# JuliaParallel/DistributedArrays.jl

Measured on NVIDIA H100. Metric: GB/s for map! and sum on Float32 DArray, higher is better.
Workload: dtype f32

## Files before the change

### distributedarrays.jl_b200/_broadcast.py

```python
from __future__ import annotations

import ctypes as C
import struct
from typing import Callable, List, Optional, Sequence, Tuple

import numpy as np

from builtins import any as builtins_any

from . import _lib
from ._darray import B200Array, DArray, dab_dtype, darray, makelocal
from .layout import shape_of
from .runtime import close_remote_reads, open_remote_reads, runtime

_RANK = {"bool": 0, "i32": 1, "i64": 2, "i128": 3, "f16": 4, "f32": 5, "f64": 6}


class _TagTypes(dict):

    def __missing__(self, tag):
        raise _lib.UnsupportedError(_lib.ERR_UNSUPPORTED, f"values of type {tag} have no array element type on the GPU backend "
                                    "(Int128 is served as the value type of mapreduce(f, op, d) only)")


_NPT = _TagTypes({"bool": np.dtype(np.bool_), "i32": np.dtype(np.int32), "i64": np.dtype(np.int64), "f32": np.dtype(np.float32),
                  "f64": np.dtype(np.float64), "c64": np.dtype(np.complex64), "c128": np.dtype(np.complex128),
                  "f16": np.dtype(np.float16)})
_TAG = {v: k for k, v in _NPT.items()}
SLICE_TRACING = [0]
_CT = {"bool": "bool", "i32": "int", "i64": "long long", "i128": "i128", "f32": "float", "f64": "double", "c64": "jl_c64", "c128": "jl_c128",
       "f16": "jl_f16"}
_COMP = {"c64": "f32", "c128": "f64"}
_CPLX_OF = {"f32": "c64", "f64": "c128"}


def _jl_name(t: str) -> str:
    return {"bool": "Bool", "i32": "Int32", "i64": "Int64", "i128": "Int128", "f16": "Float16", "f32": "Float32", "f64": "Float64"}.get(t, t)


def is_ctag(t: str) -> bool:
    return t in _COMP


def tag_of(dtype) -> str:
    dt = np.dtype(dtype)
    if dt not in _TAG:
        raise _lib.UnsupportedError(_lib.ERR_UNSUPPORTED, f"element type {dt} not served by the GPU backend")
    return _TAG[dt]


def promote(a: str, b: str) -> str:
    if a == b:
        return a
    if is_ctag(a) or is_ctag(b):
        if "i128" in (a, b):
            raise _lib.UnsupportedError(_lib.ERR_UNSUPPORTED, "Int128 values mixed with complex values are not served")
# ... 746 lines not shown
    if isinstance(a, np.ndarray) and a.ndim > 0:
        view = _bcview(a.shape, I)
        sl = a[tuple(slice(lo - 1, hi) for lo, hi in view)]
        return LocalArg(B200Array.from_numpy(rt, sl), None, tag_of(a.dtype), temp=True)
    e = Expr.wrap(a.item() if isinstance(a, np.ndarray) else a)
    return LocalArg(None, e.val, e.jt)


def _remote_args(dest_layout, args) -> List[DArray]:
    return [a for a in args if isinstance(a, DArray) and not (a.layout.pids == dest_layout.pids and a.layout.indices == dest_layout.indices)]


def _broadcast_chunks(dest: DArray, expr: Expr, args) -> DArray:
    rt = dest.rt
    fenced = open_remote_reads(rt, _remote_args(dest.layout, args), "host")
    for pid, out in dest.chunks.items():
        I = dest.layout.localindices(pid)
        largs = [_localise(rt, a, I, pid) for a in args]
        run_local(rt, expr, out, largs)
        for la in largs:
            if la.temp and la.arr is not None:
                la.arr.free()
    close_remote_reads(rt, fenced, "host")
    return dest


def _materialise_views(args):
    from ._darray import SubDArray
    out, temps = [], []
    for a in args:
        if isinstance(a, SubDArray):
            a = a.to_darray()
            temps.append(a)
        out.append(a)
    return out, temps


def broadcast_into(dest: DArray, f: Callable, *args) -> DArray:
    args, _views = _materialise_views(args)
    try:
        return _broadcast_into(dest, f, *args)
    finally:
        for v in _views:
            v.close()


def _broadcast_into(dest: DArray, f: Callable, *args) -> DArray:
    shapes = [a.dims if isinstance(a, DArray) else (a.shape if isinstance(a, np.ndarray) else ()) for a in args]
    for shp in shapes:
        for k, s in enumerate(shp):
            want = dest.dims[k] if k < len(dest.dims) else 1
            if s != 1 and s != want:
                raise _lib.DimensionMismatch(_lib.ERR_DIM_MISMATCH, f"destination axes {dest.dims} are not compatible with source axes {tuple(shp)}")
    expr = trace(f, [_arg_tag(a) for a in args])
    return _broadcast_chunks(dest, expr, args)


def broadcast(f: Callable, *args, rt=None) -> DArray:
    args, _views = _materialise_views(args)
    try:
        return _broadcast(f, *args, rt=rt)
    finally:
        for v in _views:
            v.close()


def _broadcast(f: Callable, *args, rt=None) -> DArray:
    rt = rt or next((a.rt for a in args if isinstance(a, DArray)), None) or runtime()
    shapes = [a.dims if isinstance(a, DArray) else (a.shape if isinstance(a, np.ndarray) else ()) for a in args]
    dims = _bc_shape(shapes)
    expr = trace(f, [_arg_tag(a) for a in args])
    out_dt = _NPT[expr.jt]
    dest = darray(lambda I: B200Array.empty(rt, shape_of(I), out_dt), dims, dtype=out_dt, rt=rt)
    return _broadcast_chunks(dest, expr, args)


def copy(d: DArray) -> DArray:
    from ._darray import similar
    return _broadcast_into(similar(d), lambda x: x, d)


deepcopy = copy


def drandn(dims, procs=None, dist=None, dtype=np.float64, seed: int = 1234, rt=None) -> DArray:
    from ._darray import component_dtype, drand
    dt = np.dtype(dtype)
    if dt.kind == "c":
        ct = component_dtype(dt)
        re = drandn(dims, procs, dist, dtype=ct, seed=seed, rt=rt)
        im = drandn(dims, procs, dist, dtype=ct, seed=seed + 2, rt=rt)
        from ._darray import darray_like
        out = darray_like(lambda I: B200Array.empty(re.rt, shape_of(I), dt), re, dtype=dt)
        _broadcast_into(out, lambda a, b: complex_(0.7071067811865476 * a, 0.7071067811865476 * b), re, im)
        re.close()
        im.close()
        return out
    if dt == np.dtype(np.float16):
        from ._darray import darray_like
        d64 = drandn(dims, procs, dist, dtype=np.float64, seed=seed, rt=rt)
        out = darray_like(lambda I: B200Array.empty(d64.rt, shape_of(I), dt), d64, dtype=dt)
        _broadcast_into(out, Float16, d64)
        d64.close()
        return out
    if dt.kind != "f":
        raise _lib.UnsupportedError(_lib.ERR_UNSUPPORTED, f"drandn of eltype {dt}")
    u1 = drand(dims, procs, dist, dtype=dt, seed=seed, rt=rt)
    u2 = drand(dims, procs, dist, dtype=dt, seed=seed + 1, rt=rt)
# ... 48 lines not shown
```

### distributedarrays.jl_b200/_darray.py

```python
from __future__ import annotations

import ctypes as C
import itertools
import weakref
from typing import Callable, Dict, List, Optional, Sequence, Tuple

import numpy as np

from . import _lib
from .layout import Layout, Range, default_procs, layout_from_chunk_shapes, make_layout, rlen, shape_of, slab_plan
from .runtime import Runtime, close_remote_reads, open_remote_reads, runtime

_DT = {np.dtype(np.float32): _lib.F32, np.dtype(np.float64): _lib.F64, np.dtype(np.int32): _lib.I32,
       np.dtype(np.int64): _lib.I64, np.dtype(np.bool_): _lib.U8,
       np.dtype(np.complex64): _lib.C64, np.dtype(np.complex128): _lib.C128,
       np.dtype(np.float16): _lib.F16}
_NP = {_lib.F32: np.dtype(np.float32), _lib.F64: np.dtype(np.float64), _lib.I32: np.dtype(np.int32),
       _lib.I64: np.dtype(np.int64), _lib.U8: np.dtype(np.bool_), _lib.C64: np.dtype(np.complex64), _lib.C128: np.dtype(np.complex128),
       _lib.F16: np.dtype(np.float16)}


def dab_dtype(dt) -> int:
    dt = np.dtype(dt)
    if dt not in _DT:
        raise _lib.UnsupportedError(_lib.ERR_UNSUPPORTED, f"element type {dt} is not served by the GPU backend (no host fallback)")
    return _DT[dt]


def np_dtype(code: int) -> np.dtype:
    return _NP[code]


def is_complex(dt) -> bool:
    return np.dtype(dt).kind == "c"


def component_dtype(dt) -> np.dtype:
    dt = np.dtype(dt)
    return {np.dtype(np.complex64): np.dtype(np.float32), np.dtype(np.complex128): np.dtype(np.float64)}.get(dt, dt)


def refuse_float16(what: str, *xs):
    for x in xs:
        x = getattr(x, "parent", x) if not hasattr(x, "dtype") else x
        dt = getattr(x, "dtype", None)
        if dt is not None and np.dtype(dt) == np.dtype(np.float16):
            raise _lib.UnsupportedError(_lib.ERR_UNSUPPORTED, f"{what} of Float16 data is not served (no Float16 kernel; no host fallback)")


_allowscalar = [True]


def allowscalar(flag: bool = True):
    _allowscalar[0] = bool(flag)


class B200Array:

    __slots__ = ("rt", "ptr", "shape", "dtype", "_own", "_keep", "_temp")

    def __init__(self, rt: Runtime, ptr: int, shape: Sequence[int], dtype, own: bool = True, keep=None, temp: bool = False):
        self.rt, self.ptr, self.shape, self.dtype = rt, int(ptr), tuple(int(s) for s in shape), np.dtype(dtype)
        self._own, self._keep, self._temp = own, keep, temp

    @classmethod
    def empty(cls, rt: Runtime, shape: Sequence[int], dtype, temp: bool = False) -> "B200Array":
        dtype = np.dtype(dtype)
        n = int(np.prod(shape)) if len(shape) else 1
        ptr = rt.alloc_temp(n * dtype.itemsize) if temp else rt.alloc(n * dtype.itemsize)
        return cls(rt, ptr, shape, dtype, temp=temp)

    @classmethod
    def from_numpy(cls, rt: Runtime, a: np.ndarray) -> "B200Array":
        a = np.asarray(a)
        dab_dtype(a.dtype)
        out = cls.empty(rt, a.shape, a.dtype)
        out.copy_from_host(a)
        return out

    @property
    def size(self) -> int:
        return int(np.prod(self.shape)) if len(self.shape) else 1

    @property
    def nbytes(self) -> int:
        return self.size * self.dtype.itemsize

    @property
    def ndim(self) -> int:
        return len(self.shape)

    def copy_from_host(self, a: np.ndarray, sync: bool = True):
        a = np.asarray(a, dtype=self.dtype)
        if tuple(a.shape) != self.shape:
            raise _lib.DimensionMismatch(_lib.ERR_DIM_MISMATCH, f"host array {a.shape} vs chunk {self.shape}")
        if self.size == 0:
            return
        if not a.flags.f_contiguous:
            if a.ndim == 2 and a.strides[0] == a.itemsize and a.strides[1] > 0:
                _lib.call("dab_h2d_2d", self.rt.ctx, C.c_void_p(self.ptr), a.shape[0] * a.itemsize, C.c_void_p(a.ctypes.data),
                          a.strides[1], a.shape[0] * a.itemsize, a.shape[1])
                if sync:
                    self.rt.sync()
                return
            a = np.asfortranarray(a)
        _lib.call("dab_h2d", self.rt.ctx, C.c_void_p(self.ptr), C.c_void_p(a.ctypes.data), self.nbytes)
        if sync:
            self.rt.sync()

    def to_numpy(self) -> np.ndarray:
        out = np.empty(self.shape, dtype=self.dtype, order="F")
        if self.size:
            _lib.call("dab_d2h", self.rt.ctx, C.c_void_p(out.ctypes.data), C.c_void_p(self.ptr), self.nbytes)
            self.rt.sync()
        return out

    def free(self):
        if self._own and self.ptr:
            if self._temp:
                self.rt.free_temp(self.ptr)
            else:
                self.rt.free(self.ptr)
        self.ptr = 0

    def __repr__(self):
        return f"B200Array({self.dtype}, {self.shape}, ptr=0x{self.ptr:x}, dev={self.rt.device})"


def pinned_empty(rt: Runtime, shape, dtype) -> np.ndarray:
    dtype = np.dtype(dtype)
    n = int(np.prod(shape)) if len(shape) else 1
    p = C.c_void_p()
    _lib.call("dab_host_alloc", rt.ctx, max(1, n * dtype.itemsize), C.byref(p))
    buf = (C.c_char * max(1, n * dtype.itemsize)).from_address(p.value)
    arr = np.frombuffer(buf, dtype=dtype, count=n).reshape(shape, order="F")
# ... 655 lines not shown
```

### distributedarrays.jl_b200/_mapreduce.py

```python
from __future__ import annotations

import builtins
import ctypes as C
import operator
from itertools import accumulate
from typing import Callable, Dict, Optional, Sequence, Tuple

import numpy as np

from . import _lib
from ._broadcast import Expr, broadcast, is_ctag, tag_of, trace, _NPT
from ._darray import B200Array, DArray, component_dtype, dab_dtype, is_complex, np_dtype
from .layout import Layout, ravel, reduction_passes, shape_of, unravel
from .runtime import close_remote_reads, deliver, exchange_stacks, open_remote_reads

_OPS = {"+": _lib.SUM, "add": _lib.SUM, "sum": _lib.SUM, "*": _lib.PROD, "mul": _lib.PROD, "prod": _lib.PROD, "max": _lib.MAX,
        "min": _lib.MIN}
_OPF = {operator.add: _lib.SUM, operator.mul: _lib.PROD, builtins.max: _lib.MAX, builtins.min: _lib.MIN, np.add: _lib.SUM,
        np.multiply: _lib.PROD, np.maximum: _lib.MAX, np.minimum: _lib.MIN}


def _op_code(op) -> int:
    if isinstance(op, str) and op in _OPS:
        return _OPS[op]
    if op in _OPF:
        return _OPF[op]
    raise _lib.UnsupportedError(_lib.ERR_UNSUPPORTED, f"reduction operator {op!r} is not served by a kernel (no host fallback)")


_CMPMAP = {"eq": _lib.MAP_EQ, "ne": _lib.MAP_NE, "lt": _lib.MAP_LT, "le": _lib.MAP_LE, "gt": _lib.MAP_GT, "ge": _lib.MAP_GE}
_FLIP = {"lt": "gt", "le": "ge", "gt": "lt", "ge": "le", "eq": "eq", "ne": "ne"}


def classify_map(f: Optional[Callable], dtype) -> Tuple[Optional[int], Optional[np.ndarray], Optional[Expr]]:
    if f is None:
        return _lib.MAP_ID, None, None
    tag = tag_of(dtype)
    e = trace(f, [tag])
    if e.op == "arg":
        return _lib.MAP_ID, None, e
    if is_ctag(tag):
        if len(e.args) == 1 and e.args[0].op == "arg":
            code = {"abs": _lib.MAP_ABS, "abs2": _lib.MAP_ABS2, "neg": _lib.MAP_NEG, "isnan": _lib.MAP_ISNAN}.get(e.op)
            if code is not None:
                return code, None, e
        return None, None, e
    if e.jt == tag and len(e.args) == 1 and e.args[0].op == "arg":
        code = {"abs": _lib.MAP_ABS, "abs2": _lib.MAP_ABS2, "neg": _lib.MAP_NEG}.get(e.op)
        if code is not None:
            return code, None, e
    if e.op == "mul" and e.jt == tag and builtins.all(a.op == "arg" for a in e.args):
        return _lib.MAP_ABS2, None, e
    if e.op in _CMPMAP:
        l, r = e.args

        def unpromote(side, const):
            if side.op == "convert" and side.args[0].op == "arg" and side.args[0].jt == tag and const.op == "const":
                c = const.val
                if tag in ("f32", "f16") and const.jt == "f64" and float(_NPT[tag].type(c)) == c:
                    return side.args[0], Expr("const", (), tag, c)
                if tag in ("i32", "i64") and const.jt in ("i64",) and side.jt == "i64":
                    return side.args[0], Expr("const", (), tag, c) if -2**31 <= c < 2**31 or tag == "i64" else (side, const)
            return side, const

        l, r = unpromote(l, r)
        r, l = unpromote(r, l)
        if l.op == "arg" and r.op == "const" and l.jt == tag:
            return _CMPMAP[e.op], np.asarray(r.val, dtype=np.dtype(dtype)), e
        if r.op == "arg" and l.op == "const" and r.jt == tag:
            return _CMPMAP[_FLIP[e.op]], np.asarray(l.val, dtype=np.dtype(dtype)), e
    if e.op == "isnan" and e.args[0].op == "arg":
        return _lib.MAP_ISNAN, None, e
    return None, None, e


def _result_dtype(dtype, op: int, mapc: int) -> np.dtype:
    out = C.c_int32()
    _lib.check(_lib.lib().dab_reduce_result_dtype(dab_dtype(dtype), op, mapc, C.byref(out)))
    return np.dtype(np.int64) if out.value == _lib.I64 else np_dtype(out.value)




def _gather_slots(d: DArray, launch: Callable[[int, B200Array, int], None]) -> np.ndarray:
    rt = d.rt
    wpr = rt.workers_per_rank
    slots = B200Array.empty(rt, (16 * wpr,), np.uint8, temp=True)
    try:
        for pid, ch in d.chunks.items():
            launch(pid, ch, slots.ptr + 16 * ((pid - 1) % wpr))
        if rt.world > 1:
            allslots = B200Array.empty(rt, (16 * wpr * rt.world,), np.uint8, temp=True)
            _lib.call("dab_allgather", rt.ctx, C.c_void_p(slots.ptr), C.c_void_p(allslots.ptr), 16 * wpr)
            host = allslots.to_numpy()
            allslots.free()
        else:
            host = slots.to_numpy()
    finally:
        rt.sync()
        slots.free()
    return host.view(np.uint8)


def _fold(host: np.ndarray, pids: Sequence[int], rdt: np.dtype, op: int):
    vals = np.empty(len(pids), dtype=rdt)
    for i, pid in enumerate(pids):
        vals[i] = host[16 * (pid - 1):16 * (pid - 1) + rdt.itemsize].view(rdt)[0]
    out = np.zeros(1, dtype=rdt)
    rcode = _lib.I64 if rdt == np.dtype(np.int64) else dab_dtype(rdt)
    _lib.check(_lib.lib().dab_combine_ordered(rcode, op, C.c_void_p(vals.ctypes.data), len(pids), C.c_void_p(out.ctypes.data)))
    return out[0], vals


def _int128(b: bytes) -> int:
    return int.from_bytes(b, "little", signed=True)


def wrap128(v: int) -> int:
    v &= (1 << 128) - 1
    return v - (1 << 128) if v >> 127 else v


def fold128(vals: Sequence[int], op: int) -> int:
    acc = vals[0]
    for v in vals[1:]:
        acc = wrap128(acc + v) if op == _lib.SUM else wrap128(acc * v) if op == _lib.PROD else (max(acc, v) if op == _lib.MAX else min(acc, v))
    return acc


def _check_nonempty(d: DArray, opc: int):
    if opc in (_lib.MAX, _lib.MIN):
        for pid in d.layout.pids:
# ... 45 lines not shown
        if ch.size == 0:
            return _empty_slot(rt, opc, np.dtype(np.int64) if wide else rdt, slot_ptr)
        I = d.layout.localindices(pid)
        largs = [_localise(rt, a, I, pid) for a in args]
        e, largs = split_c128_scalars(expr, largs)
        if len(largs) > 8:
            raise _lib.UnsupportedError(_lib.ERR_UNSUPPORTED, "more than 8 mapreduce arguments (a ComplexF64 scalar counts twice) are not served")
        src = codegen(e).encode()
        n = len(largs)
        dts = (C.c_int32 * n)(*[dab_dtype(NPT[la.tag]) for la in largs])
        ptrs = (C.c_void_p * n)(*[la.arr.ptr if la.arr is not None else None for la in largs])
        scal = (C.c_uint64 * n)()
        for k, la in enumerate(largs):
            if la.arr is None:
                scal[k] = int.from_bytes(np.asarray(la.scalar, dtype=NPT[la.tag]).tobytes().ljust(8, b"\0"), "little")
            elif la.temp:
                temps.append(la.arr)
        _lib.call("dab_mapreduce_expr", rt.ctx, src, val_code, opc_k, ch.size, n, dts, ptrs, scal, C.c_void_p(slot_ptr))

    try:
        host = _gather_slots(d, launch)
    finally:
        for t in temps:
            t.free()
        close_remote_reads(rt, fenced, "host")
    if wide:
        vals = [_int128(host[16 * (pid - 1):16 * pid].tobytes()) for pid in d.layout.pids]
        res = fold128(vals, opc)
        return (res, vals) if return_partials else res
    res, vals = _fold(host, d.layout.pids, rdt, opc if opc != _lib.COUNT else _lib.SUM)
    return (res, vals) if return_partials else res


def _mapreduce_all(f, op, d: DArray, return_partials: bool = False, others: Sequence = ()):
    opc = op if isinstance(op, int) else _op_code(op)
    if others:
        expr = trace(f, [tag_of(d.dtype)] + [_arg_tag_of(a) for a in others])
        return _mapreduce_expr(expr, opc, d, others, return_partials)
    mapc, param, expr = classify_map(f, d.dtype)
    if is_complex(d.dtype) and mapc is not None and not _complex_served(opc, mapc):
        if mapc == _lib.MAP_ID and opc in (_lib.MAX, _lib.MIN):
            raise TypeError(f"MethodError: no method matching isless(::{d.dtype}, ::{d.dtype}) -- complex numbers are not ordered")
        mapc = None
        if expr is None:
            expr = trace(lambda z: z, [tag_of(d.dtype)])
    if mapc is None:
        return _mapreduce_expr(expr, opc, d, (), return_partials)
    _check_nonempty(d, opc)
    rt = d.rt
    pp = C.c_void_p(param.ctypes.data) if param is not None else None
    rdt = _result_dtype(d.dtype, opc, mapc)
    if rt.workers_per_rank == 1 and d.layout.pids == rt.workers() and not return_partials:
        ch = d.chunks[rt.myid()]
        out = np.zeros(2, dtype=np.uint64)
        _lib.call("dab_mapreduce_all", rt.ctx, dab_dtype(d.dtype), opc, mapc, pp, C.c_void_p(ch.ptr), ch.size, C.c_void_p(out.ctypes.data))
        return out.view(np.uint8)[:rdt.itemsize].view(rdt)[0]
    code = dab_dtype(d.dtype)
    host = _gather_slots(d, lambda pid, ch, slot: _lib.call("dab_reduce", rt.ctx, code, opc, mapc, pp, C.c_void_p(ch.ptr), ch.size, C.c_void_p(slot)))
    res, vals = _fold(host, d.layout.pids, rdt, opc)
    return (res, vals) if return_partials else res


def _complex_served(opc: int, mapc: int) -> bool:
    out = C.c_int32()
    return _lib.lib().dab_reduce_result_dtype(_lib.C64, opc, mapc, C.byref(out)) == _lib.OK


def _arg_tag_of(a) -> str:
    from ._broadcast import _arg_tag
    return _arg_tag(a)


def reduce(op, d: DArray, dims=None, init=None):
    return mapreduce(None, op, d, dims=dims, init=init)


def mapreduce(f: Optional[Callable], op, d: DArray, *ds, dims=None, init=None, _partials: bool = False):
    from ._darray import SubDArray
    if isinstance(d, Expr):
        from . import _slices
        if _slices.tracing():
            return _slices.reduce_of_slice(f, op, d, ds, dims, init)
    if isinstance(d, SubDArray):
        tmp = d.to_darray()
        try:
            return mapreduce(f, op, tmp, *ds, dims=dims, init=init, _partials=_partials)
        finally:
            if dims is None:
                tmp.close()
    if dims is None:
        if init is not None:
            raise _lib.UnsupportedError(_lib.ERR_UNSUPPORTED, "mapreduce(f, op, d; init) without dims falls back to scalar iteration in the reference; not served")
        return _mapreduce_all(f, op, d, _partials, ds)
    if ds:
        tmp = broadcast(f, d, *ds)
        try:
            return mapreducedim(None, op, tmp, dims, init)
        finally:
            tmp.close()
    return mapreducedim(f, op, d, dims, init)


def sum(d: DArray, f: Optional[Callable] = None, dims=None):
    return mapreduce(f, "+", d, dims=dims)


def prod(d: DArray, f: Optional[Callable] = None, dims=None):
    return mapreduce(f, "*", d, dims=dims)


def maximum(d: DArray, f: Optional[Callable] = None, dims=None):
    return mapreduce(f, "max", d, dims=dims)


def minimum(d: DArray, f: Optional[Callable] = None, dims=None):
    return mapreduce(f, "min", d, dims=dims)


def _pred_reduce(opc: int, d: DArray, f: Optional[Callable]):
    from ._darray import SubDArray
    if isinstance(d, SubDArray):
        tmp = d.to_darray()
        try:
            return _pred_reduce(opc, tmp, f)
        finally:
            tmp.close()
    if f is None:
        if d.dtype != np.dtype(np.bool_):
            raise TypeError("TypeError: non-boolean used in boolean context")
        return _mapreduce_all(None, opc, d)
    mapc, param, e = classify_map(f, d.dtype)
# ... 343 lines not shown
```

### distributedarrays.jl_b200/csrc/dab_comm.cu

```cuda
#include <dlfcn.h>
#include <nccl.h>

#include "dab_common.cuh"
#include "dab_scalar_ops.cuh"

namespace {

struct NcclApi {
    void* handle = nullptr;
    ncclResult_t (*GetUniqueId)(ncclUniqueId*) = nullptr;
    ncclResult_t (*CommInitRank)(ncclComm_t*, int, ncclUniqueId, int) = nullptr;
    ncclResult_t (*CommDestroy)(ncclComm_t) = nullptr;
    ncclResult_t (*AllGather)(const void*, void*, size_t, ncclDataType_t, ncclComm_t, cudaStream_t) = nullptr;
    ncclResult_t (*AllReduce)(const void*, void*, size_t, ncclDataType_t, ncclRedOp_t, ncclComm_t, cudaStream_t) = nullptr;
    ncclResult_t (*Send)(const void*, size_t, ncclDataType_t, int, ncclComm_t, cudaStream_t) = nullptr;
    ncclResult_t (*Recv)(void*, size_t, ncclDataType_t, int, ncclComm_t, cudaStream_t) = nullptr;
    ncclResult_t (*GroupStart)() = nullptr;
    ncclResult_t (*GroupEnd)() = nullptr;
    const char* (*GetErrorString)(ncclResult_t) = nullptr;
    const char* (*GetLastError)(ncclComm_t) = nullptr;
    bool ok = false;
    char why[256] = "";
};

// ... 70 lines not shown
            __threadfence_system();
            break;
        }
    }
    __threadfence_system();
}

template <typename T>
__global__ void __launch_bounds__(256) accumulate_stack_kernel(T* __restrict__ y, size_t n, T beta, int beta_mode, T alpha, int alpha_one,
                                                              const T* __restrict__ stack, size_t stride, int count) {
    for (size_t i = (size_t)blockIdx.x * 256 + threadIdx.x; i < n; i += (size_t)gridDim.x * 256) {
        T v = beta_mode == 0 ? T(0) : (beta_mode == 1 ? y[i] : jl::mul(y[i], beta));
        for (int j = 0; j < count; ++j) {
            const T r = stack[(size_t)j * stride + i];
            v = jl::add(v, alpha_one ? r : jl::mul(alpha, r));
        }
        y[i] = v;
    }
}

}

extern "C" {

int32_t dab_comm_unique_id(void* id128) {
    NEED_NCCL(nullptr);
    if (!id128) return dab_fail(nullptr, DAB_ERR_ARG, "null id");
    static_assert(sizeof(ncclUniqueId) == 128, "ncclUniqueId is 128 bytes");
    ncclUniqueId id;
    DAB_NCCL(nullptr, api.GetUniqueId(&id));
    memcpy(id128, &id, 128);
    return DAB_OK;
}

int32_t dab_comm_init_rank(dab_ctx* ctx, const void* id128, int32_t rank, int32_t nranks) {
    DAB_ENTER(ctx);
    NEED_NCCL(ctx);
    DAB_REQUIRE(ctx, id128 && nranks >= 1 && rank >= 0 && rank < nranks && nranks <= DAB_MAX_RANKS, DAB_ERR_ARG,
                "dab_comm_init_rank: bad rank %d / nranks %d", rank, nranks);
    DAB_REQUIRE(ctx, !ctx->comm, DAB_ERR_ARG, "communicator already initialised");
    ncclUniqueId id;
    memcpy(&id, id128, 128);
    ncclComm_t comm;
    DAB_NCCL(ctx, api.CommInitRank(&comm, nranks, id, rank));
    ctx->comm = (void*)comm;
    ctx->rank = rank;
    ctx->nranks = nranks;
    return DAB_OK;
}

int32_t dab_comm_destroy(dab_ctx* ctx) {
    if (!ctx || !ctx->comm) return DAB_OK;
    NcclApi& api = nccl();
    cudaSetDevice(ctx->device);
    const int32_t st = dab_flush_pending(ctx);
    cudaStreamSynchronize(ctx->stream);
    if (api.ok) api.CommDestroy((ncclComm_t)ctx->comm);
    ctx->comm = nullptr;
    ctx->rank = 0;
    ctx->nranks = 1;
    return st;
}

int32_t dab_allgather(dab_ctx* ctx, const void* send_dev, void* recv_dev, size_t nbytes_per_rank) {
    DAB_ENTER(ctx);
    NEED_COMM(ctx);
    DAB_NCCL(ctx, api.AllGather(send_dev, recv_dev, nbytes_per_rank, ncclInt8, (ncclComm_t)ctx->comm, ctx->stream));
    ctx->launches++;
    return DAB_OK;
}

int32_t dab_allreduce(dab_ctx* ctx, int32_t dtype, int32_t op, const void* send_dev, void* recv_dev, size_t count) {
    DAB_ENTER(ctx);
    NEED_COMM(ctx);
    ncclDataType_t dt;
    switch (dtype) {
        case DAB_F32: dt = ncclFloat32; break;
        case DAB_F64: dt = ncclFloat64; break;
        case DAB_I32: dt = ncclInt32; break;
        case DAB_I64: dt = ncclInt64; break;
        case DAB_U8: dt = ncclUint8; break;
        default: return dab_fail(ctx, DAB_ERR_ARG, "dab_allreduce: bad dtype %d", dtype);
    }
    ncclRedOp_t ro;
    switch (op) {
        case DAB_SUM: ro = ncclSum; break;
        case DAB_PROD: ro = ncclProd; break;
        case DAB_MAX: ro = ncclMax; break;
        case DAB_MIN: ro = ncclMin; break;
        default: return dab_fail(ctx, DAB_ERR_ARG, "dab_allreduce: bad op %d", op);
    }
    DAB_NCCL(ctx, api.AllReduce(send_dev, recv_dev, count, dt, ro, (ncclComm_t)ctx->comm, ctx->stream));
    ctx->launches++;
    return DAB_OK;
}

int32_t dab_group_start(dab_ctx* ctx) {
    DAB_ENTER(ctx);
    NEED_COMM(ctx);
    DAB_NCCL(ctx, api.GroupStart());
    return DAB_OK;
}
int32_t dab_group_end(dab_ctx* ctx) {
    DAB_ENTER(ctx);
    NEED_COMM(ctx);
    DAB_NCCL(ctx, api.GroupEnd());
    ctx->launches++;
// ... 51 lines not shown
        ctx->launches++;
        src = ctx->gather_slots;
    }
    DAB_CUDA(ctx, cudaMemcpyAsync(ctx->host_slot, src, (size_t)P * 16, cudaMemcpyDeviceToHost, ctx->stream));
    DAB_CUDA(ctx, cudaStreamSynchronize(ctx->stream));
    unsigned char tmp[DAB_MAX_RANKS * 16];
    size_t es = dab_dtype_size(rdt);
    for (int i = 0; i < P; ++i) memcpy(tmp + (size_t)i * es, (const char*)ctx->host_slot + (size_t)i * 16, es);
    unsigned char res[16] = {0};
    st = dab_combine_ordered(rdt, op, tmp, (size_t)P, res);
    if (st != DAB_OK) return dab_fail(ctx, st, "%s", dab_last_error(nullptr));
    memset(out_host, 0, es > 8 ? es : 8);
    memcpy(out_host, res, es);
    return DAB_OK;
}

int32_t dab_mailbox_create(dab_ctx* ctx, void* handle64) {
    DAB_ENTER(ctx);
    DAB_REQUIRE(ctx, handle64, DAB_ERR_ARG, "dab_mailbox_create: null handle");
    if (!ctx->mailbox) {
        DAB_CUDA(ctx, cudaMalloc(&ctx->mailbox, DAB_MBOX_BYTES));
        DAB_CUDA(ctx, cudaMemset(ctx->mailbox, 0, DAB_MBOX_BYTES));
    }
    cudaIpcMemHandle_t h;
    DAB_CUDA(ctx, cudaIpcGetMemHandle(&h, ctx->mailbox));
    memcpy(handle64, &h, 64);
    return DAB_OK;
}

int32_t dab_mailbox_attach(dab_ctx* ctx, const void* handles, int32_t rank, int32_t nranks) {
    DAB_ENTER(ctx);
    DAB_REQUIRE(ctx, handles && nranks >= 1 && nranks <= DAB_MAX_RANKS && rank >= 0 && rank < nranks, DAB_ERR_ARG, "dab_mailbox_attach: bad arguments");
    DAB_REQUIRE(ctx, ctx->mailbox, DAB_ERR_ARG, "dab_mailbox_attach: call dab_mailbox_create first");
    DAB_REQUIRE(ctx, ctx->mbox_ranks == 0, DAB_ERR_ARG, "mailboxes already attached");
    for (int j = 0; j < nranks; ++j) {
        if (j == rank) {
            ctx->peer_mbox_host[j] = ctx->mailbox;
            continue;
        }
        cudaIpcMemHandle_t h;
        memcpy(&h, (const char*)handles + (size_t)j * 64, 64);
        DAB_CUDA(ctx, cudaIpcOpenMemHandle(&ctx->peer_mbox_host[j], h, cudaIpcMemLazyEnablePeerAccess));
    }
    DAB_CUDA(ctx, cudaMalloc((void**)&ctx->peer_mbox_dev, sizeof(void*) * DAB_MAX_RANKS));
    DAB_CUDA(ctx, cudaMemcpy(ctx->peer_mbox_dev, ctx->peer_mbox_host, sizeof(void*) * nranks, cudaMemcpyHostToDevice));
    ctx->rank = rank;
    ctx->mbox_ranks = nranks;
    ctx->mbox_seq = 0;
    return DAB_OK;
}

int32_t dab_mailbox_detach(dab_ctx* ctx) {
    if (!ctx) return DAB_OK;
    cudaSetDevice(ctx->device);
    const int32_t st = dab_flush_pending(ctx);
    for (int j = 0; j < ctx->mbox_ranks; ++j)
        if (j != ctx->rank && ctx->peer_mbox_host[j]) cudaIpcCloseMemHandle(ctx->peer_mbox_host[j]);
    if (ctx->peer_mbox_dev) cudaFree(ctx->peer_mbox_dev);
    if (ctx->mailbox) cudaFree(ctx->mailbox);
    ctx->peer_mbox_dev = nullptr;
    ctx->mailbox = nullptr;
    ctx->mbox_ranks = 0;
    cudaGetLastError();
    return st;
}


int32_t dab_peer_barrier(dab_ctx* ctx) {
    DAB_ENTER(ctx);
    if (ctx->mbox_ranks <= 1) return DAB_OK;
    volatile unsigned long long* status = (volatile unsigned long long*)((char*)ctx->host_slot + (DAB_MAX_RANKS + 1) * 16);
    const unsigned long long seq = ++ctx->barrier_seq;
    peer_barrier_kernel<<<1, DAB_MAX_RANKS, 0, ctx->stream>>>(ctx->peer_mbox_dev, ctx->rank, ctx->mbox_ranks, seq,
                                                             (unsigned long long)ctx->opt_combine_timeout_ms * 1000000ull, status);
    DAB_LAUNCHED(ctx);
    return DAB_OK;
}

int32_t dab_accumulate_stack(dab_ctx* ctx, int32_t dtype, void* y, size_t n, const void* beta, const void* alpha, const void* stack, size_t stride,
                             int32_t count) {
    DAB_ENTER(ctx);
    if (n == 0) return DAB_OK;
    DAB_REQUIRE(ctx, y && beta && alpha && (stack || count == 0) && count >= 0, DAB_ERR_ARG, "dab_accumulate_stack: bad argument");
    const int grid = dab_grid_for(ctx, (n + 255) / 256, 8);
#define ACC(T)                                                                                                                       \
    {                                                                                                                                \
        const T b = *(const T*)beta, a = *(const T*)alpha, zero = 0, one = 1;                                                        \
        accumulate_stack_kernel<T><<<grid, 256, 0, ctx->stream>>>((T*)y, n, b, b == zero ? 0 : (b == one ? 1 : 2), a, a == one,     \
                                                                   (const T*)stack, stride, count);                                  \
        DAB_LAUNCHED(ctx);                                                                                                           \
        return DAB_OK;                                                                                                               \
    }
    switch (dtype) {
        case DAB_F32: ACC(float)
        case DAB_F64: ACC(double)
        case DAB_I32: ACC(int32_t)
        case DAB_I64: ACC(long long)
        default: return dab_fail(ctx, DAB_ERR_UNSUPPORTED, "dab_accumulate_stack: dtype %d", dtype);
    }
#undef ACC
}

int32_t dab_ipc_get_handle(dab_ctx* ctx, const void* dptr, void* handle64) {
    DAB_ENTER(ctx);
    DAB_REQUIRE(ctx, dptr && handle64, DAB_ERR_ARG, "dab_ipc_get_handle: null pointer");
    static_assert(sizeof(cudaIpcMemHandle_t) == 64, "cudaIpcMemHandle_t is 64 bytes");
    cudaIpcMemHandle_t h;
// ... 34 lines not shown
```

### distributedarrays.jl_b200/csrc/dab_common.cuh

```cuda
#pragma once
#include <cuda_runtime.h>

#include <cstdint>
#include <cstdio>
#include <cstring>

#include "../../include/dab200.h"

#define DAB_MAX_REDUCE_BLOCKS 262144
#define DAB_SLOT_BYTES 64
#define DAB_MAX_RANKS 64

struct dab_pending_affine {
    int active;
    int32_t dtype;
    void* y;
    const void* x;
    size_t n;
    unsigned char a[8], b[8];
};

struct dab_ctx {
    int device;
    int sm_count;
    cudaStream_t stream;
    void* block_partials;
    unsigned int* counter;
    void* result_slot;
    void* gather_slots;
    void* host_slot;
    void* dim_scratch;
    size_t dim_scratch_bytes;
    uint64_t launches;
    void* comm;
    int rank, nranks;
    void* mailbox;
    void** peer_mbox_dev;
    void* peer_mbox_host[DAB_MAX_RANKS];
    int mbox_ranks;
    unsigned long long mbox_seq;
    unsigned long long barrier_seq;
    int fuse_op;
    struct dab_alloc_cache* cache;
    void* sort_dev;
    size_t sort_dev_bytes;
    void* stage[2];
    cudaEvent_t stage_ev[2];
    void* sort_host;
    unsigned long long sort_epoch;
    void* scan_dev;
    size_t scan_dev_bytes;
    unsigned long long scan_epoch;
    unsigned long long scan_tickets;
    void* scan_scratch;
    size_t scan_scratch_bytes;
    long long opt_combine_timeout_ms;
    int opt_ew_tma;
    dab_pending_affine pending;
    int defer_off;
    char err[512];
};

extern thread_local char dab_tls_err[512];

int32_t dab_fail(dab_ctx* ctx, int32_t status, const char* fmt, ...);
int32_t dab_fail_cuda(dab_ctx* ctx, cudaError_t e, const char* what, const char* file, int line);

#define DAB_CUDA(ctx, call)                                                             \
    do {                                                                                \
        cudaError_t e__ = (call);                                                       \
        if (e__ != cudaSuccess) return dab_fail_cuda((ctx), e__, #call, __FILE__, __LINE__); \
    } while (0)

#define DAB_REQUIRE(ctx, cond, status, ...)                          \
    do {                                                             \
        if (!(cond)) return dab_fail((ctx), (status), __VA_ARGS__);  \
    } while (0)

int32_t dab_flush_pending(dab_ctx* ctx);

#define DAB_FLUSH(ctx)                                    \
    do {                                                  \
        if ((ctx)->pending.active) {                      \
            int32_t st__ = dab_flush_pending(ctx);        \
            if (st__ != DAB_OK) return st__;              \
        }                                                 \
    } while (0)

#define DAB_ENTER(ctx)                                                      \
    do {                                                                    \
        if ((ctx) == nullptr) return dab_fail(nullptr, DAB_ERR_ARG, "null ctx"); \
        DAB_CUDA((ctx), cudaSetDevice((ctx)->device));                      \
        DAB_FLUSH(ctx);                                                     \
    } while (0)

#define DAB_ENTER_NOFLUSH(ctx)                                              \
    do {                                                                    \
        if ((ctx) == nullptr) return dab_fail(nullptr, DAB_ERR_ARG, "null ctx"); \
        DAB_CUDA((ctx), cudaSetDevice((ctx)->device));                      \
    } while (0)

#define DAB_LAUNCHED(ctx)                          \
    do {                                           \
        (ctx)->launches++;                         \
        DAB_CUDA((ctx), cudaGetLastError());       \
    } while (0)

int32_t dab_scratch_grow(dab_ctx* ctx, void** buf, size_t* have, size_t bytes, bool zero);

static inline size_t dab_dtype_size(int32_t dt) {
    switch (dt) {
        case DAB_F32: return 4;
        case DAB_F64: return 8;
        case DAB_I32: return 4;
        case DAB_I64: return 8;
        case DAB_U8: return 1;
        case DAB_C64: return 8;
        case DAB_C128: return 16;
        case DAB_F16: return 2;
        default: return 0;
    }
}

#define DAB_MBOX_SLOT 32
#define DAB_MBOX_BARRIER_OFFSET (2 * DAB_MAX_RANKS * DAB_MBOX_SLOT)
#define DAB_MBOX_BYTES (DAB_MBOX_BARRIER_OFFSET + DAB_MAX_RANKS * 8)
struct FusedComm {
    void* const* peers;
    void* host_out;
    unsigned long long seq;
    unsigned long long timeout_ns;
    int rank, nranks, op;
};

__device__ __forceinline__ unsigned long long dab_globaltimer_ns() {
    unsigned long long t;
    asm volatile("mov.u64 %0, %globaltimer;" : "=l"(t));
    return t;
}
__device__ __forceinline__ int4 ld_stream(const int4* p) { return __ldcs(p); }
__device__ __forceinline__ void st_stream(int4* p, int4 v) { __stcs(p, v); }

template <typename T>
struct alignas(16) Pack {
    static constexpr int N = 16 / sizeof(T);
    T v[N];
};

template <typename T>
struct alignas(2 * sizeof(T)) Cplx {
    T re, im;
};
// ... 95 lines not shown
```

### distributedarrays.jl_b200/csrc/dab_core.cu

```cuda
#include <cstdarg>
#include <cstdlib>
#include <map>
#include <mutex>
#include <new>
#include <thread>
#include <unordered_map>

#include "dab_common.cuh"

thread_local char dab_tls_err[512] = "";

struct dab_alloc_cache {
    std::unordered_map<void*, size_t> live;
    std::multimap<size_t, void*> free_blocks;
    size_t cached_bytes = 0;
    static constexpr size_t kMaxBlock = 16ull << 30;
    static constexpr size_t kMaxCached = 32ull << 30;
};

int dab_resident_ctas(const void* kernel, int threads) {
    static std::mutex mu;
    static std::unordered_map<const void*, int> cache;
    std::lock_guard<std::mutex> lk(mu);
    auto it = cache.find(kernel);
// ... 79 lines not shown
    if (device < 0 || device >= n) return dab_fail(nullptr, DAB_ERR_ARG, "device %d out of range (have %d)", device, n);
    dab_ctx* ctx = new (std::nothrow) dab_ctx();
    if (!ctx) return dab_fail(nullptr, DAB_ERR_NOMEM, "host allocation failed");
    memset(ctx, 0, sizeof(*ctx));
    ctx->device = device;
    ctx->rank = 0;
    ctx->nranks = 1;
    ctx->fuse_op = -1;
    ctx->opt_combine_timeout_ms = 120000;
    ctx->cache = new (std::nothrow) dab_alloc_cache();
#define INIT_CUDA(call)                                                     \
    do {                                                                    \
        cudaError_t e__ = (call);                                           \
        if (e__ != cudaSuccess) {                                           \
            int32_t st = dab_fail_cuda(nullptr, e__, #call, __FILE__, __LINE__); \
            delete ctx;                                                     \
            return st;                                                      \
        }                                                                   \
    } while (0)
    INIT_CUDA(cudaSetDevice(device));
    cudaDeviceProp prop;
    INIT_CUDA(cudaGetDeviceProperties(&prop, device));
    if (prop.major != 9 || prop.minor != 0) {
        delete ctx;
        return dab_fail(nullptr, DAB_ERR_UNSUPPORTED, "device %d is sm_%d%d; libdab200 is built for sm_90a only", device,
                        prop.major, prop.minor);
    }
    ctx->sm_count = prop.multiProcessorCount;
    INIT_CUDA(cudaStreamCreateWithFlags(&ctx->stream, cudaStreamNonBlocking));
    {
        cudaMemPool_t pool;
        INIT_CUDA(cudaDeviceGetDefaultMemPool(&pool, device));
        unsigned long long keep = ~0ull;
        INIT_CUDA(cudaMemPoolSetAttribute(pool, cudaMemPoolAttrReleaseThreshold, &keep));
    }
    INIT_CUDA(cudaMalloc(&ctx->block_partials, ((size_t)DAB_MAX_REDUCE_BLOCKS + DAB_MAX_REDUCE_BLOCKS / 256 + 16) * 16));
    INIT_CUDA(cudaMalloc((void**)&ctx->counter, (DAB_MAX_REDUCE_BLOCKS / 256 + 16) * 4));
    INIT_CUDA(cudaMemsetAsync(ctx->counter, 0, (DAB_MAX_REDUCE_BLOCKS / 256 + 16) * 4, ctx->stream));
    INIT_CUDA(cudaMalloc(&ctx->result_slot, DAB_SLOT_BYTES));
    INIT_CUDA(cudaMalloc(&ctx->gather_slots, (size_t)DAB_MAX_RANKS * 16));
    INIT_CUDA(cudaHostAlloc(&ctx->host_slot, (size_t)(DAB_MAX_RANKS + 2) * 16, cudaHostAllocDefault));
    INIT_CUDA(cudaStreamSynchronize(ctx->stream));
    memset(ctx->host_slot, 0, (size_t)(DAB_MAX_RANKS + 2) * 16);
#undef INIT_CUDA
    *out = ctx;
    return DAB_OK;
}

int32_t dab_comm_destroy(dab_ctx* ctx);
int32_t dab_mailbox_detach(dab_ctx* ctx);

int32_t dab_shutdown(dab_ctx* ctx) {
    if (!ctx) return DAB_OK;
    cudaSetDevice(ctx->device);
    const int32_t st = dab_flush_pending(ctx);
    cudaStreamSynchronize(ctx->stream);
    if (ctx->comm) dab_comm_destroy(ctx);
    cudaFree(ctx->block_partials);
    cudaFree(ctx->counter);
    cudaFree(ctx->result_slot);
    cudaFree(ctx->gather_slots);
    if (ctx->dim_scratch) cudaFree(ctx->dim_scratch);
    if (ctx->sort_dev) cudaFree(ctx->sort_dev);
    if (ctx->scan_dev) cudaFree(ctx->scan_dev);
    if (ctx->scan_scratch) cudaFree(ctx->scan_scratch);
    if (ctx->sort_host) cudaFreeHost(ctx->sort_host);
    for (int b = 0; b < 2; ++b)
        if (ctx->stage[b]) {
            cudaFreeHost(ctx->stage[b]);
            cudaEventDestroy(ctx->stage_ev[b]);
        }
    if (ctx->cache) {
        for (auto& kv : ctx->cache->free_blocks) cudaFree(kv.second);
        delete ctx->cache;
        ctx->cache = nullptr;
    }
    dab_mailbox_detach(ctx);
    cudaFreeHost(ctx->host_slot);
    cudaStreamDestroy(ctx->stream);
    delete ctx;
    return st;
}

int32_t dab_sync(dab_ctx* ctx) {
    DAB_ENTER(ctx);
    DAB_CUDA(ctx, cudaStreamSynchronize(ctx->stream));
    volatile unsigned long long* status = (volatile unsigned long long*)((char*)ctx->host_slot + (DAB_MAX_RANKS + 1) * 16);
    if (*status != 0) {
        *status = 0;
        return dab_fail(ctx, DAB_ERR_NCCL, "device-side peer barrier timed out waiting for another rank (did every rank make the same collective call?)");
    }
    return DAB_OK;
}

int32_t dab_device_info(dab_ctx* ctx, int32_t* device, int32_t* sm_count, size_t* free_bytes, size_t* total_bytes) {
    DAB_ENTER(ctx);
    size_t f = 0, t = 0;
    DAB_CUDA(ctx, cudaMemGetInfo(&f, &t));
    if (device) *device = ctx->device;
    if (sm_count) *sm_count = ctx->sm_count;
    if (free_bytes) *free_bytes = f + (ctx->cache ? ctx->cache->cached_bytes : 0);
    if (total_bytes) *total_bytes = t;
    return DAB_OK;
}

int32_t dab_stream(dab_ctx* ctx, void** stream) {
    DAB_ENTER(ctx);
    DAB_REQUIRE(ctx, stream, DAB_ERR_ARG, "null stream out-pointer");
    ctx->defer_off = 1;
    *stream = (void*)ctx->stream;
    return DAB_OK;
}

int32_t dab_set_option(dab_ctx* ctx, const char* key, int64_t value) {
    if (!ctx || !key) return dab_fail(ctx, DAB_ERR_ARG, "null argument");
    if (ctx->pending.active) {
        DAB_CUDA(ctx, cudaSetDevice(ctx->device));
        DAB_FLUSH(ctx);
    }
    if (strcmp(key, "ew_tma") == 0) {
        ctx->opt_ew_tma = value != 0;
        return DAB_OK;
    }
    if (strcmp(key, "combine_timeout_ms") == 0) {
        if (value < 1) return dab_fail(ctx, DAB_ERR_ARG, "combine_timeout_ms must be >= 1");
        ctx->opt_combine_timeout_ms = value;
        return DAB_OK;
    }
    return dab_fail(ctx, DAB_ERR_ARG, "dab_set_option: unknown key %s", key);
}

int32_t dab_launch_count(dab_ctx* ctx, uint64_t* launches) {
    if (!ctx || !launches) return dab_fail(ctx, DAB_ERR_ARG, "null argument");
    if (ctx->pending.active) {
        DAB_CUDA(ctx, cudaSetDevice(ctx->device));
        DAB_FLUSH(ctx);
    }
    *launches = ctx->launches;
    return DAB_OK;
}

int32_t dab_event_create(dab_ctx* ctx, void** event) {
    DAB_ENTER(ctx);
    DAB_REQUIRE(ctx, event, DAB_ERR_ARG, "null event out-pointer");
    cudaEvent_t ev;
    DAB_CUDA(ctx, cudaEventCreate(&ev));
    *event = (void*)ev;
    return DAB_OK;
}
int32_t dab_event_record(dab_ctx* ctx, void* event) {
    DAB_ENTER(ctx);
    DAB_CUDA(ctx, cudaEventRecord((cudaEvent_t)event, ctx->stream));
    return DAB_OK;
}
int32_t dab_event_elapsed_ms(dab_ctx* ctx, void* start, void* stop, float* ms) {
    DAB_ENTER(ctx);
    DAB_REQUIRE(ctx, ms, DAB_ERR_ARG, "null ms");
    DAB_CUDA(ctx, cudaEventSynchronize((cudaEvent_t)stop));
    DAB_CUDA(ctx, cudaEventElapsedTime(ms, (cudaEvent_t)start, (cudaEvent_t)stop));
    return DAB_OK;
}
int32_t dab_event_destroy(dab_ctx* ctx, void* event) {
    DAB_ENTER(ctx);
    DAB_CUDA(ctx, cudaEventDestroy((cudaEvent_t)event));
    return DAB_OK;
}

int32_t dab_alloc(dab_ctx* ctx, size_t nbytes, void** dptr) {
    DAB_ENTER(ctx);
    DAB_REQUIRE(ctx, dptr, DAB_ERR_ARG, "null dptr out-pointer");
    *dptr = nullptr;
    if (nbytes == 0) nbytes = 16;
    dab_alloc_cache* c = ctx->cache;
    if (c && nbytes <= dab_alloc_cache::kMaxBlock) {
        const size_t rounded = (nbytes + 511) & ~(size_t)511;
        auto it = c->free_blocks.find(rounded);
        if (it != c->free_blocks.end()) {
            *dptr = it->second;
            c->free_blocks.erase(it);
            c->cached_bytes -= rounded;
        } else {
            cudaError_t e = cudaMalloc(dptr, rounded);
            if (e == cudaErrorMemoryAllocation) {
                cudaGetLastError();
                DAB_CUDA(ctx, cudaStreamSynchronize(ctx->stream));
                for (auto& kv : c->free_blocks) cudaFree(kv.second);
                c->free_blocks.clear();
                c->cached_bytes = 0;
// ... 189 lines not shown
    dab_generate_kernel<T, Gen><<<(unsigned)grid, 256, 0, ctx->stream>>>(x, n, gen);
    DAB_LAUNCHED(ctx);
    return DAB_OK;
}

extern "C" {

int32_t dab_fill(dab_ctx* ctx, int32_t dtype, void* x, size_t n, const void* value) {
    DAB_ENTER(ctx);
    DAB_REQUIRE(ctx, (x || n == 0) && value, DAB_ERR_ARG, "dab_fill: null pointer");
    switch (dtype) {
        case DAB_F32: return launch_generate(ctx, (float*)x, n, FillGen<float>{*(const float*)value});
        case DAB_F64: return launch_generate(ctx, (double*)x, n, FillGen<double>{*(const double*)value});
        case DAB_I32: return launch_generate(ctx, (int32_t*)x, n, FillGen<int32_t>{*(const int32_t*)value});
        case DAB_I64: return launch_generate(ctx, (long long*)x, n, FillGen<long long>{*(const long long*)value});
        case DAB_U8: return launch_generate(ctx, (uint8_t*)x, n, FillGen<uint8_t>{*(const uint8_t*)value});
        case DAB_F16: {
            DAB_REQUIRE(ctx, (uintptr_t)x % 2 == 0, DAB_ERR_ARG, "dab_fill: Float16 data needs 2-byte alignment");
            FillGen<Half> g;
            memcpy(&g.v, value, 2);
            return launch_generate(ctx, (Half*)x, n, g);
        }
        case DAB_C64:
        case DAB_C128: {
            const size_t es = dab_dtype_size(dtype);
            DAB_REQUIRE(ctx, (uintptr_t)x % es == 0, DAB_ERR_ARG, "dab_fill: complex dtype %d needs %d-byte aligned data", dtype, (int)es);
            if (dtype == DAB_C64) {
                FillGen<Cplx<float>> g;
                memcpy(&g.v, value, 8);
                return launch_generate(ctx, (Cplx<float>*)x, n, g);
            }
            FillGen<Cplx<double>> g;
            memcpy(&g.v, value, 16);
            return launch_generate(ctx, (Cplx<double>*)x, n, g);
        }
        default: return dab_fail(ctx, DAB_ERR_ARG, "dab_fill: bad dtype %d", dtype);
    }
}

int32_t dab_rand_u01(dab_ctx* ctx, int32_t dtype, void* x, size_t n, uint64_t seed, uint64_t global_offset) {
    DAB_ENTER(ctx);
    DAB_REQUIRE(ctx, x || n == 0, DAB_ERR_ARG, "dab_rand_u01: null pointer");
    switch (dtype) {
        case DAB_F32: return launch_generate(ctx, (float*)x, n, RandGen<float>{seed, global_offset});
        case DAB_F64: return launch_generate(ctx, (double*)x, n, RandGen<double>{seed, global_offset});
        case DAB_F16:
            DAB_REQUIRE(ctx, (uintptr_t)x % 2 == 0, DAB_ERR_ARG, "dab_rand_u01: Float16 data needs 2-byte alignment");
            return launch_generate(ctx, (Half*)x, n, RandGenF16{seed, global_offset});
        default: return dab_fail(ctx, DAB_ERR_UNSUPPORTED, "dab_rand_u01: dtype %d (F32/F64/F16 only)", dtype);
    }
}

}
```

Measured before the change: 4078.

## Cache broadcast plans, add affine fast path, and trim host call overhead

```diff
diff --git a/distributedarrays.jl_b200/_broadcast.py b/distributedarrays.jl_b200/_broadcast.py
--- a/distributedarrays.jl_b200/_broadcast.py
+++ b/distributedarrays.jl_b200/_broadcast.py
@@ -2,6 +2,7 @@
 
 import ctypes as C
 import struct
+import types
 from typing import Callable, List, Optional, Sequence, Tuple
 
 import numpy as np
@@ -854,8 +855,90 @@
             want = dest.dims[k] if k < len(dest.dims) else 1
             if s != 1 and s != want:
                 raise _lib.DimensionMismatch(_lib.ERR_DIM_MISMATCH, f"destination axes {dest.dims} are not compatible with source axes {tuple(shp)}")
-    expr = trace(f, [_arg_tag(a) for a in args])
+    expr, affine = _plan(f, [_arg_tag(a) for a in args], dest.dtype)
+    if affine is not None and type(args[0]) is DArray and _same_chunks(args[0], dest):
+        return _affine_chunks(dest, args[0], affine)
     return _broadcast_chunks(dest, expr, args)
+
+
+_PLANS: dict = {}
+_PLANS_MAX = 256
+
+
+def _value_key(v):
+    t = type(v)
+    if t is float:
+        return t, struct.pack("<d", v)
+    if t is int or t is bool:
+        return t, v
+    if t is complex:
+        return t, struct.pack("<dd", v.real, v.imag)
+    if isinstance(v, np.generic) and t.__module__ == "numpy" and v.dtype.kind in "biufc":
+        return t, v.tobytes()
+    return None
+
+
+def _plan_key(f, tags, out_dtype):
+    if type(f) is not types.FunctionType or f.__code__.co_names or f.__kwdefaults__:
+        return None
+    key = [f.__code__, tuple(tags), out_dtype]
+    for cell in f.__closure__ or ():
+        try:
+            k = _value_key(cell.cell_contents)
+        except ValueError:
+            return None
+        if k is None:
+            return None
+        key.append(k)
+    for v in f.__defaults__ or ():
+        k = _value_key(v)
+        if k is None:
+            return None
+        key.append(k)
+    return tuple(key)
+
+
+def _affine_args(expr: Expr, tags, out_dtype):
+    out_tag = _TAG.get(np.dtype(out_dtype))
+    if out_tag is None or out_tag == "bool" or expr.jt != out_tag or len(tags) != 1 or tags[0] != out_tag:
+        return None
+    if uses_complex(expr) or is_ctag(out_tag) or uses_tag(expr, "f16") or out_tag == "f16" or not all(_only_arg0(expr)):
+        return None
+    ab = match_affine(expr)
+    if ab is None:
+        return None
+    a, b = np.asarray(ab[0], dtype=out_dtype), np.asarray(ab[1], dtype=out_dtype)
+    return dab_dtype(out_dtype), a.ctypes.data, b.ctypes.data, (a, b)
+
+
+def _plan(f: Callable, tags, out_dtype):
+    key = _plan_key(f, tags, out_dtype)
+    plan = _PLANS.get(key) if key is not None else None
+    if plan is None:
+        expr = trace(f, tags)
+        plan = (expr, _affine_args(expr, tags, out_dtype))
+        if key is not None:
+            if len(_PLANS) >= _PLANS_MAX:
+                _PLANS.clear()
+            _PLANS[key] = plan
+    return plan
+
+
+def _same_chunks(x: DArray, dest: DArray) -> bool:
+    lx, ld = x.layout, dest.layout
+    return (lx is ld or (lx.pids == ld.pids and lx.indices == ld.indices)) and x.chunks.keys() == dest.chunks.keys()
+
+
+def _affine_chunks(dest: DArray, x: DArray, affine) -> DArray:
+    rt = dest.rt
+    code, pa, pb, _ = affine
+    for pid, out in dest.chunks.items():
+        n = out.size
+        if n == 0:
+            continue
+        _lib.call("dab_affine", rt.ctx, code, out.ptr, x.chunks[pid].ptr, pa, pb, n)
+        rt.last_kernel = "dab_affine"
+    return dest
 
 
 def broadcast(f: Callable, *args, rt=None) -> DArray:
diff --git a/distributedarrays.jl_b200/_darray.py b/distributedarrays.jl_b200/_darray.py
--- a/distributedarrays.jl_b200/_darray.py
+++ b/distributedarrays.jl_b200/_darray.py
@@ -2,6 +2,7 @@
 
 import ctypes as C
 import itertools
+import math
 import weakref
 from typing import Callable, Dict, List, Optional, Sequence, Tuple
 
@@ -80,7 +81,7 @@
 
     @property
     def size(self) -> int:
-        return int(np.prod(self.shape)) if len(self.shape) else 1
+        return math.prod(self.shape)
 
     @property
     def nbytes(self) -> int:
diff --git a/distributedarrays.jl_b200/_mapreduce.py b/distributedarrays.jl_b200/_mapreduce.py
--- a/distributedarrays.jl_b200/_mapreduce.py
+++ b/distributedarrays.jl_b200/_mapreduce.py
@@ -10,7 +10,7 @@
 
 from . import _lib
 from ._broadcast import Expr, broadcast, is_ctag, tag_of, trace, _NPT
-from ._darray import B200Array, DArray, component_dtype, dab_dtype, is_complex, np_dtype
+from ._darray import B200Array, DArray, SubDArray, component_dtype, dab_dtype, is_complex, np_dtype
 from .layout import Layout, ravel, reduction_passes, shape_of, unravel
 from .runtime import close_remote_reads, deliver, exchange_stacks, open_remote_reads
 
@@ -74,10 +74,17 @@
     return None, None, e
 
 
+_RESULT_DTYPES: Dict[Tuple[np.dtype, int, int], np.dtype] = {}
+
+
 def _result_dtype(dtype, op: int, mapc: int) -> np.dtype:
-    out = C.c_int32()
-    _lib.check(_lib.lib().dab_reduce_result_dtype(dab_dtype(dtype), op, mapc, C.byref(out)))
-    return np.dtype(np.int64) if out.value == _lib.I64 else np_dtype(out.value)
+    key = (np.dtype(dtype), op, mapc)
+    rdt = _RESULT_DTYPES.get(key)
+    if rdt is None:
+        out = C.c_int32()
+        _lib.check(_lib.lib().dab_reduce_result_dtype(dab_dtype(dtype), op, mapc, C.byref(out)))
+        rdt = _RESULT_DTYPES[key] = np.dtype(np.int64) if out.value == _lib.I64 else np_dtype(out.value)
+    return rdt
 
 
 
@@ -229,9 +236,9 @@
     rdt = _result_dtype(d.dtype, opc, mapc)
     if rt.workers_per_rank == 1 and d.layout.pids == rt.workers() and not return_partials:
         ch = d.chunks[rt.myid()]
-        out = np.zeros(2, dtype=np.uint64)
-        _lib.call("dab_mapreduce_all", rt.ctx, dab_dtype(d.dtype), opc, mapc, pp, C.c_void_p(ch.ptr), ch.size, C.c_void_p(out.ctypes.data))
-        return out.view(np.uint8)[:rdt.itemsize].view(rdt)[0]
+        out = (C.c_uint64 * 2)()
+        _lib.call("dab_mapreduce_all", rt.ctx, dab_dtype(d.dtype), opc, mapc, pp, ch.ptr, ch.size, out)
+        return np.frombuffer(out, dtype=rdt, count=1)[0]
     code = dab_dtype(d.dtype)
     host = _gather_slots(d, lambda pid, ch, slot: _lib.call("dab_reduce", rt.ctx, code, opc, mapc, pp, C.c_void_p(ch.ptr), ch.size, C.c_void_p(slot)))
     res, vals = _fold(host, d.layout.pids, rdt, opc)
@@ -253,7 +260,6 @@
 
 
 def mapreduce(f: Optional[Callable], op, d: DArray, *ds, dims=None, init=None, _partials: bool = False):
-    from ._darray import SubDArray
     if isinstance(d, Expr):
         from . import _slices
         if _slices.tracing():
diff --git a/distributedarrays.jl_b200/csrc/dab_comm.cu b/distributedarrays.jl_b200/csrc/dab_comm.cu
--- a/distributedarrays.jl_b200/csrc/dab_comm.cu
+++ b/distributedarrays.jl_b200/csrc/dab_comm.cu
@@ -146,7 +146,7 @@
 int32_t dab_comm_destroy(dab_ctx* ctx) {
     if (!ctx || !ctx->comm) return DAB_OK;
     NcclApi& api = nccl();
-    cudaSetDevice(ctx->device);
+    dab_set_device(ctx->device);
     const int32_t st = dab_flush_pending(ctx);
     cudaStreamSynchronize(ctx->stream);
     if (api.ok) api.CommDestroy((ncclComm_t)ctx->comm);
@@ -304,7 +304,7 @@
 
 int32_t dab_mailbox_detach(dab_ctx* ctx) {
     if (!ctx) return DAB_OK;
-    cudaSetDevice(ctx->device);
+    dab_set_device(ctx->device);
     const int32_t st = dab_flush_pending(ctx);
     for (int j = 0; j < ctx->mbox_ranks; ++j)
         if (j != ctx->rank && ctx->peer_mbox_host[j]) cudaIpcCloseMemHandle(ctx->peer_mbox_host[j]);
diff --git a/distributedarrays.jl_b200/csrc/dab_common.cuh b/distributedarrays.jl_b200/csrc/dab_common.cuh
--- a/distributedarrays.jl_b200/csrc/dab_common.cuh
+++ b/distributedarrays.jl_b200/csrc/dab_common.cuh
@@ -63,6 +63,8 @@
 
 extern thread_local char dab_tls_err[512];
 
+cudaError_t dab_set_device(int device);
+
 int32_t dab_fail(dab_ctx* ctx, int32_t status, const char* fmt, ...);
 int32_t dab_fail_cuda(dab_ctx* ctx, cudaError_t e, const char* what, const char* file, int line);
 
@@ -75,6 +77,12 @@
 #define DAB_REQUIRE(ctx, cond, status, ...)                          \
     do {                                                             \
         if (!(cond)) return dab_fail((ctx), (status), __VA_ARGS__);  \
+    } while (0)
+
+#define DAB_SET_DEVICE(ctx, dev)                                                                               \
+    do {                                                                                                       \
+        cudaError_t e__ = dab_set_device(dev);                                                                 \
+        if (e__ != cudaSuccess) return dab_fail_cuda((ctx), e__, "cudaSetDevice(" #dev ")", __FILE__, __LINE__); \
     } while (0)
 
 int32_t dab_flush_pending(dab_ctx* ctx);
@@ -90,14 +98,14 @@
 #define DAB_ENTER(ctx)                                                      \
     do {                                                                    \
         if ((ctx) == nullptr) return dab_fail(nullptr, DAB_ERR_ARG, "null ctx"); \
-        DAB_CUDA((ctx), cudaSetDevice((ctx)->device));                      \
+        DAB_SET_DEVICE((ctx), (ctx)->device);                               \
         DAB_FLUSH(ctx);                                                     \
     } while (0)
 
 #define DAB_ENTER_NOFLUSH(ctx)                                              \
     do {                                                                    \
         if ((ctx) == nullptr) return dab_fail(nullptr, DAB_ERR_ARG, "null ctx"); \
-        DAB_CUDA((ctx), cudaSetDevice((ctx)->device));                      \
+        DAB_SET_DEVICE((ctx), (ctx)->device);                               \
     } while (0)
 
 #define DAB_LAUNCHED(ctx)                          \
diff --git a/distributedarrays.jl_b200/csrc/dab_core.cu b/distributedarrays.jl_b200/csrc/dab_core.cu
--- a/distributedarrays.jl_b200/csrc/dab_core.cu
+++ b/distributedarrays.jl_b200/csrc/dab_core.cu
@@ -155,7 +155,7 @@
 
 int32_t dab_shutdown(dab_ctx* ctx) {
     if (!ctx) return DAB_OK;
-    cudaSetDevice(ctx->device);
+    dab_set_device(ctx->device);
     const int32_t st = dab_flush_pending(ctx);
     cudaStreamSynchronize(ctx->stream);
     if (ctx->comm) dab_comm_destroy(ctx);
@@ -218,7 +218,7 @@
 int32_t dab_set_option(dab_ctx* ctx, const char* key, int64_t value) {
     if (!ctx || !key) return dab_fail(ctx, DAB_ERR_ARG, "null argument");
     if (ctx->pending.active) {
-        DAB_CUDA(ctx, cudaSetDevice(ctx->device));
+        DAB_SET_DEVICE(ctx, ctx->device);
         DAB_FLUSH(ctx);
     }
     if (strcmp(key, "ew_tma") == 0) {
@@ -236,7 +236,7 @@
 int32_t dab_launch_count(dab_ctx* ctx, uint64_t* launches) {
     if (!ctx || !launches) return dab_fail(ctx, DAB_ERR_ARG, "null argument");
     if (ctx->pending.active) {
-        DAB_CUDA(ctx, cudaSetDevice(ctx->device));
+        DAB_SET_DEVICE(ctx, ctx->device);
         DAB_FLUSH(ctx);
     }
     *launches = ctx->launches;
@@ -532,3 +532,13 @@
 }
 
 }
+
+static thread_local int dab_tls_device = -1;
+
+cudaError_t dab_set_device(int device) {
+    int cur = -1;
+    if (dab_tls_device == device && cudaGetDevice(&cur) == cudaSuccess && cur == device) return cudaSuccess;
+    const cudaError_t e = cudaSetDevice(device);
+    dab_tls_device = e == cudaSuccess ? device : -1;
+    return e;
+}
```

New measurement: 4198 (median of 6 runs). +3.0%, better.
